# tigert1998/ray-tracing-cuda

Hardware: AMD Instinct MI355X
Metric: Mrays/s (higher is better)
Workload: dtype f32

## Files before the change

### ray-tracing-cuda_amd/csrc/closest_hit.h

```cpp
#pragma once

#ifdef RTMI_CHECK_MARGINS
__device__ inline bool aabb_hit_reference(const BvhNode &nd, V3 o, V3 d, double t_from, double t_to) {
  const float oo[3] = {o.x, o.y, o.z}, dd[3] = {d.x, d.y, d.z};
  for (int i = 0; i < 3; i++) {
    if (dd[i] == 0.f) continue;
    for (int s = 0; s < 2; s++) {
      const float tf = ((s == 0 ? nd.mn[i] : nd.mx[i]) - oo[i]) / dd[i];
      const double t = (double)tf;
      if (t != t || fabs(t) == (double)INFINITY) continue;
      if (!(t_from <= t && t <= t_to)) continue;
      const float pt[3] = {oo[0] + (float)t * dd[0], oo[1] + (float)t * dd[1], oo[2] + (float)t * dd[2]};
      bool inside = true;
      for (int a = 0; a < 3; a++)
        if (a != i && !(nd.mn[a] <= pt[a] && pt[a] <= nd.mx[a])) inside = false;
      if (inside) return true;
    }
  }
  return false;
}
template <typename T>
__device__ inline bool bvh_reference_walk(const SceneDev &sc, const BvhRec &br, V3 o, V3 d, T &t_to, int &face, float &fu,
                                          float &fv) {
  int stk_node[kRefDepthMax + 2], stk_first[kRefDepthMax + 2], stk_n[kRefDepthMax + 2];
  int sp = 1;
  stk_node[0] = br.root, stk_first[0] = 0, stk_n[0] = br.n_faces;
  bool hit = false;
  while (sp > 0) {
    sp--;
    const int node = stk_node[sp], first = stk_first[sp], n = stk_n[sp];
    const BvhNode nd = sc.nodes[node];
    if (node != br.root && !aabb_hit_reference(nd, o, d, 1e-3, (double)t_to)) continue;
    if (nd.right < 0) {
      for (int i = 0; i < n; i++) {
        const int fi = sc.face_of_orig[br.face_base + first + i];
        const FaceRec &f = sc.faces[fi];
        float t = 0.f, u = 0.f, v = 0.f;
        if (tri_test<T>(mk(f.p0[0], f.p0[1], f.p0[2]), mk(f.e1[0], f.e1[1], f.e1[2]), mk(f.e2[0], f.e2[1], f.e2[2]), o, d,
                        t_to, t, u, v))
          t_to = (T)t, face = fi, fu = u, fv = v, hit = true;
      }
    } else if (sp + 2 <= kRefDepthMax + 2) {
      const int mid = (n - 1) / 2;
      stk_node[sp] = nd.right, stk_first[sp] = first + mid + 1, stk_n[sp] = n - mid - 1;
      stk_node[sp + 1] = nd.left, stk_first[sp + 1] = first, stk_n[sp + 1] = mid + 1;
      sp += 2;
    }
  }
  return hit;
}
#endif

template <uint32_t M>
__device__ __forceinline__ bool load_tri_pts(const SceneDev &sc, const float4 *s_tris, int rec, int which, V3 &p0, V3 &e1, V3 &e2) {
  float4 qa, qb, qc;
  bool present;
  if ((M & PIN_LDS_TABLES) || s_tris != nullptr) {
    const float4 *pp = s_tris + (size_t)rec * 3;
    qa = load_lds<float4>(pp), qb = load_lds<float4>(pp + 1), qc = load_lds<float4>(pp + 2);
    present = !(__float_as_int(qc.y) & TRIPTS_ABSENT);
  } else {
    const float4 *pp = reinterpret_cast<const float4 *>(sc.tris + rec);
    qa = load_global<float4>(pp), qb = load_global<float4>(pp + 1), qc = load_global<float4>(pp + 2);
    const float4 qd = load_global<float4>(pp + 3);
    present = which == 0 || (__float_as_int(qd.y) & TRI_SECOND);
  }
  p0 = mk(qa.x, qa.y, qa.z), e1 = mk(qa.w, qb.x, qb.y), e2 = mk(qb.z, qb.w, qc.x);
  return present;
}

template <uint32_t F, bool OCC = false, uint32_t M = 0>
__device__ __forceinline__ Hit closest_hit(const SceneDev &sc, const BvhNode *s_nodes, int lds_nodes, const int *s_paths,
                                           int lds_paths, const float4 *s_tris, int *ll, uint16_t *cands, int *wl,
                                           unsigned long long *overflow, V3 o, V3 d, bool live, bool count_work
#ifdef RTMI_STATS
                                           , MeshStats &st
#endif
                                           , double t_start = INFINITY, double t_stop = INFINITY, bool *uncertain = nullptr
) {
  constexpr bool DT = (F & F_SPHERE) != 0;
  typedef typename TSel<DT>::type T;
  bool ok = false;
  T t_to = OCC ? (T)t_start : (T)INFINITY;
#define RTMI_DECIDED (OCC && ok && t_to <= (T)t_stop)
  uint32_t win = ID_NONE;
  int32_t aux = 0;
  int32_t work = 0;
  float bu = 0.f, bv = 0.f;

  double sa = 0.0, sa2 = 0.0;
  float saf = 0.f;
  if (F & F_SPHERE) {
    float la = len3(d);
    saf = la * la;
    sa = (double)saf;
    sa2 = 2 * sa;
  }

  const int lane = (int)(threadIdx.x & 63u);
  const bool det_safe = (M & PIN_DET_SAFE) || sc.det_safe != 0;
  constexpr bool SLAB = culls_by_slab(M);
  const bool cull_list = (F & F_TRIS) && ((M & PIN_LDS_TABLES) || (ll != nullptr && sc.n_pairs >= kCullMinPairs));
  V3 cull_inv = splat(0.f), cull_klo = splat(0.f), cull_khi = splat(0.f);
  if ((F & F_TRIS) && cull_list) {
    const float ix = __builtin_amdgcn_rcpf(d.x), iy = __builtin_amdgcn_rcpf(d.y), iz = __builtin_amdgcn_rcpf(d.z);
    cull_inv = mk(fabsf(d.x) < 1e-30f ? copysignf(1e30f, d.x) : ix, fabsf(d.y) < 1e-30f ? copysignf(1e30f, d.y) : iy,
                  fabsf(d.z) < 1e-30f ? copysignf(1e30f, d.z) : iz);
    if (SLAB) {
      cull_klo = mk(-o.x * cull_inv.x, -o.y * cull_inv.y, -o.z * cull_inv.z);
    } else {
      const float delta = MESH_DIST_SLACK * (fmaxf(fmaxf(fabsf(o.x), fabsf(o.y)), fabsf(o.z)) + sc.list_mag);
      cull_klo = mk(-(o.x + delta) * cull_inv.x, -(o.y + delta) * cull_inv.y, -(o.z + delta) * cull_inv.z);
      cull_khi = mk(-(o.x - delta) * cull_inv.x, -(o.y - delta) * cull_inv.y, -(o.z - delta) * cull_inv.z);
    }
  }

  for (int ri = 0; ri < sc.n_runs; ri++) {
    if (OCC) {
      live = live && !RTMI_DECIDED;
      if (__builtin_amdgcn_ballot_w64(live) == 0ull) break;
    }
    const i32x4 rv = load_run(sc.runs, ri);
    Run run;
    run.kind = rv[0], run.first = rv[1], run.count = rv[2], run.pad = rv[3];
    if (live && run.kind == RUN_SKY) {
      const T ts = (T)1e9f;
      bool hit = ts <= t_to;
      bool acc = hit && (!ok || ts < t_to);
      ok = ok || acc;
      t_to = acc ? ts : t_to;
      win = acc ? make_id(RUN_SKY, 0) : win;
    }
    if ((F & F_TRIS) && run.kind == RUN_TRIS && cull_list) {
      const int pair0 = run.first >> 1;
      const float lo0 = T_FROM_F * kTimeLo;
      for (int c0 = 0; c0 < run.count; c0 += 32) {
        if (OCC && __builtin_amdgcn_ballot_w64(live && !RTMI_DECIDED) == 0ull) break;
        const int nc = run.count - c0 < 32 ? run.count - c0 : 32;
        const float hi0 = (float)t_to * kTimeHi + kTimeAbs;
        uint32_t mask = 0u;
        RTMI_STAT2(const unsigned long long tc0 = stat_now();)
#define RTMI_CULL_PAIR(bx)                                                                                                      \
  {                                                                                                                             \
    const float t0x = __builtin_fmaf(bx[0], cull_inv.x, cull_klo.x), t1x = __builtin_fmaf(bx[3], cull_inv.x, cull_khi.x); \
    const float t0y = __builtin_fmaf(bx[1], cull_inv.y, cull_klo.y), t1y = __builtin_fmaf(bx[4], cull_inv.y, cull_khi.y); \
    const float t0z = __builtin_fmaf(bx[2], cull_inv.z, cull_klo.z), t1z = __builtin_fmaf(bx[5], cull_inv.z, cull_khi.z); \
    const float en = fmaxf(fmaxf(fminf(t0x, t1x), fminf(t0y, t1y)), fminf(t0z, t1z));                                            \
    const float le = fminf(fminf(fmaxf(t0x, t1x), fmaxf(t0y, t1y)), fmaxf(t0z, t1z));                                            \
    cull_step(mask, fmaxf(lo0, en), fminf(hi0, le));                                                                            \
  }
#define RTMI_CULL_SLAB(bx)                                                                                                      \
  {                                                                                                                             \
    const float tcx = __builtin_fmaf(bx[0], cull_inv.x, cull_klo.x), tcy = __builtin_fmaf(bx[1], cull_inv.y, cull_klo.y),       \
                tcz = __builtin_fmaf(bx[2], cull_inv.z, cull_klo.z);                                                            \
    const float nx = __builtin_fmaf(-bx[3], fabsf(cull_inv.x), tcx), fx = __builtin_fmaf(bx[3], fabsf(cull_inv.x), tcx);        \
    const float ny = __builtin_fmaf(-bx[4], fabsf(cull_inv.y), tcy), fy = __builtin_fmaf(bx[4], fabsf(cull_inv.y), tcy);        \
    const float nz = __builtin_fmaf(-bx[5], fabsf(cull_inv.z), tcz), fz = __builtin_fmaf(bx[5], fabsf(cull_inv.z), tcz);        \
    const float en = fmaxf(fmaxf(nx, ny), nz), le = fminf(fminf(fx, fy), fz);                                                   \
    cull_step_nlt(mask, fminf(hi0, le), fmaxf(lo0, en));                                                                        \
  }
#define RTMI_CULL_ONE(bx)  \
  if (SLAB) RTMI_CULL_SLAB(bx) else RTMI_CULL_PAIR(bx)
        const PairBox *const recs = sc.pair_boxes;
        f32x8 A = load_pair_box(recs, pair0 + c0), B;
        int i = 0;
        for (; i + 1 < nc; i += 2) {
          __builtin_amdgcn_s_waitcnt(0xc07f);
          __builtin_amdgcn_sched_barrier(0);
          B = load_pair_box(recs, pair0 + c0 + i + 1);
          __builtin_amdgcn_sched_barrier(0);
          RTMI_CULL_ONE(A)
          __builtin_amdgcn_s_waitcnt(0xc07f);
          __builtin_amdgcn_sched_barrier(0);
          A = load_pair_box(recs, pair0 + c0 + i + 2);
          __builtin_amdgcn_sched_barrier(0);
          RTMI_CULL_ONE(B)
        }
        if (i < nc) {
          __builtin_amdgcn_s_waitcnt(0xc07f);
          __builtin_amdgcn_sched_barrier(0);
          RTMI_CULL_ONE(A)
        }
#undef RTMI_CULL_ONE
#undef RTMI_CULL_SLAB
#undef RTMI_CULL_PAIR
        mask = __brev(mask) >> (32 - nc);
        if (!live) mask = 0u;
        if (OCC && RTMI_DECIDED) mask = 0u;
        RTMI_STAT2(const unsigned long long tc1 = stat_now(); st.cyc[5] += tc1 - tc0;)
        RTMI_STAT(st.cull_bits += (unsigned)__popcll(__builtin_amdgcn_ballot_w64(true)) * 0u; { unsigned pc = __builtin_popcount(mask); for (int off = 32; off > 0; off >>= 1) pc += __shfl_down(pc, off); st.cull_bits += __builtin_amdgcn_readfirstlane(pc); } st.cull_rays += (unsigned)__popcll(__builtin_amdgcn_ballot_w64(true));)
#ifndef RTMI_OWN_FIRST
#define RTMI_OWN_FIRST 1
#endif
#if RTMI_OWN_FIRST
        if (__builtin_amdgcn_ballot_w64(mask != 0u) != 0ull) {
          if (mask != 0u) {
            const int bit = __builtin_ctz(mask);
            mask &= mask - 1u;
            const int rec = 2 * (pair0 + c0 + bit);
            V3 p0, e1, e2, p1, e1b, e2b;
            (void)load_tri_pts<M>(sc, s_tris, rec, 0, p0, e1, e2);
            const bool second = load_tri_pts<M>(sc, s_tris, rec + 1, 1, p1, e1b, e2b);
            float ta = 0.f, ua = 0.f, va = 0.f, tb = 0.f, ub = 0.f, vb = 0.f;
            const bool hit_a = tri_test_flat<T>(p0, e1, e2, cross3(d, e2), o, d, t_to, ta, ua, va, det_safe);
            bool hit_b = false;
            if (second) hit_b = tri_test_flat<T>(p1, e1b, e2b, cross3(d, e2b), o, d, t_to, tb, ub, vb, det_safe) && !hit_a;
            const float t = hit_a ? ta : tb;
            const bool acc = (hit_a || hit_b) && (!ok || (T)t < t_to);
            ok = ok || acc;
            t_to = acc ? (T)t : t_to;
            win = acc ? make_id(RUN_TRIS, run.first + 2 * (c0 + bit) + (hit_a ? 0 : 1)) : win;
            if (F & F_TEX) {
              bu = acc ? (hit_a ? ua : ub) : bu;
              bv = acc ? (hit_a ? va : vb) : bv;
            }
          }
        }
        if (OCC && RTMI_DECIDED) mask = 0u;
#endif
        {
          constexpr int RW = (F & F_TEX) ? 6 : 2;
          int *tasks = ll + 64 * 8, *results = ll + 64 * 8 + kListTasks(F);
          const int cnt = __builtin_popcount(mask);
          const int base = wave_prefix_excl(cnt);
          if (cnt != 0) {
            int *rr = ll + lane * 8;
            int w3 = 0, w7 = 0;
            if (DT) {
              const double td = (double)t_to;
              w3 = __double2loint(td), w7 = __double2hiint(td);
            } else {
              w3 = __float_as_int((float)t_to);
            }
            *reinterpret_cast<int4 *>(rr) = make_int4(__float_as_int(o.x), __float_as_int(o.y), __float_as_int(o.z), w3);
            *reinterpret_cast<int4 *>(rr + 4) = make_int4(__float_as_int(d.x), __float_as_int(d.y), __float_as_int(d.z), w7);
          }
          bool todo = cnt != 0;
          while (__builtin_amdgcn_ballot_w64(todo) != 0ull) {
            RTMI_STAT(st.cull_iters++;)
            const int lo_t = __builtin_amdgcn_readlane(base, __builtin_ctzll(__builtin_amdgcn_ballot_w64(todo)));
            const bool now = todo && base + cnt - lo_t <= kListTasks(F);
            const int n_now = __builtin_amdgcn_readlane(base + cnt, 63 - __builtin_clzll(__builtin_amdgcn_ballot_w64(now))) - lo_t;
            RTMI_STAT(st.nnow_hist[(n_now - 1) >> 5 < 5 ? (n_now - 1) >> 5 : 5]++;)
            if (now) {
              int k = base - lo_t;
              for (uint32_t m = mask; m != 0u; m &= m - 1u) tasks[k++] = (lane << 5) | __builtin_ctz(m);
            }
            wave_lds_fence();
            for (int t0 = 0; t0 < 2 * n_now; t0 += 64) {
              const int ti = t0 + lane;
              if (ti < 2 * n_now) {
                const int w = tasks[ti >> 1], which = ti & 1;
                const int *orr = ll + (w >> 5) * 8;
                const float4 r0 = *reinterpret_cast<const float4 *>(orr), r1 = *reinterpret_cast<const float4 *>(orr + 4);
                T t0_to;
                if (DT) {
                  t0_to = (T)__hiloint2double(__float_as_int(r1.w), __float_as_int(r0.w));
                } else {
                  t0_to = (T)r0.w;
                }
                const V3 ro = mk(r0.x, r0.y, r0.z), rd = mk(r1.x, r1.y, r1.z);
                V3 p0, e1, e2;
                const bool present = load_tri_pts<M>(sc, s_tris, 2 * (pair0 + c0 + (w & 31)) + which, which, p0, e1, e2);
                float tt = 0.f, uu = 0.f, vv = 0.f;
                bool hit = false;
                if (present) hit = tri_test_flat<T>(p0, e1, e2, cross3(rd, e2), ro, rd, t0_to, tt, uu, vv, det_safe);
                int *res = results + (ti >> 1) * RW;
                res[which] = hit ? __float_as_int(tt) : (int)0xffffffff;
                if (F & F_TEX) res[2 + 2 * which] = __float_as_int(uu), res[3 + 2 * which] = __float_as_int(vv);
              }
            }
            wave_lds_fence();
            RTMI_STAT2(const unsigned long long tc2 = stat_now();)
            if (now) {
              int k = base - lo_t;
              for (uint32_t m = mask; m != 0u; m &= m - 1u, k++) {
                const int tri = run.first + 2 * (c0 + __builtin_ctz(m));
                const int *res = results + k * RW;
                const int ia = res[0], ib = res[1];
                const float ta = __int_as_float(ia), tb = __int_as_float(ib);
                const bool hit_a = ia != (int)0xffffffff && (T)ta <= t_to;
                const bool hit_b = !hit_a && ib != (int)0xffffffff && (T)tb <= t_to;
                const float t = hit_a ? ta : tb;
                const bool acc = (hit_a || hit_b) && (!ok || (T)t < t_to);
                ok = ok || acc;
                t_to = acc ? (T)t : t_to;
                win = acc ? make_id(RUN_TRIS, tri + (hit_a ? 0 : 1)) : win;
                if (F & F_TEX) {
                  bu = acc ? __int_as_float(hit_a ? res[2] : res[4]) : bu;
                  bv = acc ? __int_as_float(hit_a ? res[3] : res[5]) : bv;
                }
              }
              todo = false;
            }
            wave_lds_fence();
            RTMI_STAT2(st.cyc[7] += stat_now() - tc2;)
          }
        }
        RTMI_STAT2(st.cyc[6] += stat_now() - tc1;)
      }
    } else if ((F & F_TRIS) && live && run.kind == RUN_TRIS) {
      const HotTri *base = sc.tris + run.first;
      f32x16 A = load_hot_tri(base, 0);
      for (int i = 0; i < run.count; i++) {
        if (OCC && __builtin_amdgcn_ballot_w64(!RTMI_DECIDED) == 0ull) break;
        __builtin_amdgcn_s_waitcnt(0xc07f);
        __builtin_amdgcn_sched_barrier(0);
        const f32x16 B = load_hot_tri(base, 2 * i + 1);
        __builtin_amdgcn_sched_barrier(0);
        float t = 0.f, u = 0.f, v = 0.f;
        const V3 pv_a = cross3(d, mk(A[6], A[7], A[8]));
        const bool hit_a = tri_test_flat<T>(mk(A[0], A[1], A[2]), mk(A[3], A[4], A[5]), mk(A[6], A[7], A[8]), pv_a, o, d,
                                            t_to, t, u, v, det_safe);
        {
          bool acc = hit_a && (!ok || (T)t < t_to);
          ok = ok || acc;
          t_to = acc ? (T)t : t_to;
          win = acc ? make_id(RUN_TRIS, run.first + 2 * i) : win;
          if (F & F_TEX) {
            bu = acc ? u : bu;
            bv = acc ? v : bv;
          }
        }
        __builtin_amdgcn_s_waitcnt(0xc07f);
        __builtin_amdgcn_sched_barrier(0);
        A = load_hot_tri(base, 2 * i + 2);
        __builtin_amdgcn_sched_barrier(0);
        if (__float_as_int(B[13]) & TRI_SECOND) {
          V3 pv_b = pv_a;
          if (!(__float_as_int(B[13]) & TRI_SAME_E2)) pv_b = cross3(d, mk(B[6], B[7], B[8]));
          bool hit_b = tri_test_flat<T>(mk(B[0], B[1], B[2]), mk(B[3], B[4], B[5]), mk(B[6], B[7], B[8]), pv_b, o, d,
                                        t_to, t, u, v, det_safe);
          hit_b = hit_b && !hit_a;
          bool acc = hit_b && (!ok || (T)t < t_to);
          ok = ok || acc;
          t_to = acc ? (T)t : t_to;
          win = acc ? make_id(RUN_TRIS, run.first + 2 * i + 1) : win;
          if (F & F_TEX) {
            bu = acc ? u : bu;
            bv = acc ? v : bv;
          }
        }
      }
    }
    bool grouped_done = false;
    if ((F & F_SGROUP) && run.kind == RUN_SPHERE && run.pad >= 0 && cands != nullptr) {
      const int n_groups = (run.count + kSphGroupSize - 1) / kSphGroupSize;
      uint16_t *my_cands = cands + lane * kSphCand;
      int *tasks = ll + 64 * 8, *results = ll + 64 * 8 + kListTasks(F);
      int ccnt = 0;
      bool have = false;
      double best_v = 0.0;
      int best_idx = 0;
      {
        int *rr = ll + lane * 8;
        *reinterpret_cast<int4 *>(rr) = make_int4(__float_as_int(o.x), __float_as_int(o.y), __float_as_int(o.z), __float_as_int(saf));
        *reinterpret_cast<int4 *>(rr + 4) = make_int4(__float_as_int(d.x), __float_as_int(d.y), __float_as_int(d.z), 0);
      }
      const float sdelta = kSphDistSlack * fmaxf(fmaxf(fabsf(o.x), fabsf(o.y)), fabsf(o.z));
      const float six = __builtin_amdgcn_rcpf(d.x), siy = __builtin_amdgcn_rcpf(d.y), siz = __builtin_amdgcn_rcpf(d.z);
      const V3 s_inv = mk(fabsf(d.x) < 1e-30f ? copysignf(1e30f, d.x) : six, fabsf(d.y) < 1e-30f ? copysignf(1e30f, d.y) : siy,
                          fabsf(d.z) < 1e-30f ? copysignf(1e30f, d.z) : siz);
      const V3 s_klo = mk(-(o.x + sdelta) * s_inv.x, -(o.y + sdelta) * s_inv.y, -(o.z + sdelta) * s_inv.z);
      const V3 s_khi = mk(-(o.x - sdelta) * s_inv.x, -(o.y - sdelta) * s_inv.y, -(o.z - sdelta) * s_inv.z);
      const float s_lo0 = T_FROM_F * kTimeLo, s_hi0 = (float)t_to * kTimeHi + kTimeAbs;
      const int member0 = __float_as_int(load_sph_group(sc.sph_groups, run.pad)[6]);
      auto flush = [&]() {
        const int cnt = ccnt;
        const int base = wave_prefix_excl(cnt);
        bool todo = cnt != 0;
        while (__builtin_amdgcn_ballot_w64(todo) != 0ull) {
          const int lo_t = __builtin_amdgcn_readlane(base, __builtin_ctzll(__builtin_amdgcn_ballot_w64(todo)));
          const bool now = todo && base + cnt - lo_t <= kListTasks(F);
          const int n_now = __builtin_amdgcn_readlane(base + cnt, 63 - __builtin_clzll(__builtin_amdgcn_ballot_w64(now))) - lo_t;
          if (now)
            for (int j = 0; j < cnt; j++) tasks[base - lo_t + j] = (lane << 16) | (int)my_cands[j];
          wave_lds_fence();
          for (int t0 = 0; t0 < n_now; t0 += 64) {
            const int ti = t0 + lane;
            if (ti < n_now) {
              const int w = tasks[ti];
              const int *orr = ll + (w >> 16) * 8;
              const float4 r0 = *reinterpret_cast<const float4 *>(orr), r1 = *reinterpret_cast<const float4 *>(orr + 4);
              const SphMember *mp = sc.sph_members + member0 + (w & 0xffff);
              const float4 m0 = *reinterpret_cast<const float4 *>(mp);
              const int4 m1 = *reinterpret_cast<const int4 *>(reinterpret_cast<const char *>(mp) + 16);
              const double r2 = __hiloint2double(m1.w, m1.z);
              const V3 ro = mk(r0.x, r0.y, r0.z), rd = mk(r1.x, r1.y, r1.z);
              const double tsa = (double)r0.w, tsa2 = 2 * tsa;
              const V3 oc = ro - mk(m0.x, m0.y, m0.z);
              const double b = (double)(2.0f * dot3(rd, oc));
              const float lc = len3(oc);
              const double c = (double)(lc * lc) - r2;
              const double disc = b * b - 4 * tsa * c;
              double v = __hiloint2double(0x7ff80000, 0);
              if (!(disc < 0)) {
                const double sq = sqrt(disc);
                const double t1 = (-b - sq) / tsa2;
                if (1e-3 <= t1) {
                  v = t1;
                } else {
// ... 386 lines not shown
```

### ray-tracing-cuda_amd/csrc/kernels.h

```cpp
#pragma once
#include <hip/hip_runtime.h>
#include <stdint.h>

#include "../../include/rtmi.h"
#include "scene_dev.h"

#define RTMI_KERNEL_MAX_DEPTH 64

namespace rtmi {

int64_t frame_pixel_of(const FrameDev &fr, int rank, int64_t q);

hipError_t launch_rng_init(uint64_t seed, const FrameDev &fr, const uint32_t *d_jump, uint32_t *d_states,
                           hipStream_t stream, int64_t first = -1);

uint32_t pick_variant(uint32_t features);
int render_occupancy(uint32_t variant, const SceneDev &sc, const FrameDev &fr, int threads, bool fast_path = false);
struct RenderTuning {
  int schedule;
  int blocks_per_cu;
  int threads;
  int sparse_stride;
  int exclusive;
  int outlier_x10;
  int head_pct[3];
  int probe_spp;
  int promote;
  int first_pass;
  int cost_probe;
  int lane_stride;
  int plan;
  int prio_every;
  int fast_path;
  int head_classes;
  int first_prio;
  int fetch_batch, fetch_batch_first;
};

enum : uint32_t {
  PIN_NIBBLE_IDS = 1u << 0,
  PIN_LDS_TABLES = 1u << 1,
  PIN_UNSIGNED = 1u << 2,
  PIN_DET_SAFE = 1u << 3,
  PIN_POW2_FRAME = 1u << 4,
  PIN_EVERY_LANE = 1u << 5,
  PIN_PRIORITIES = 1u << 6,
  PIN_CHAINS = 1u << 7,
  PIN_QUEUE = 1u << 8,
};
constexpr uint32_t kFastCommon = PIN_NIBBLE_IDS | PIN_LDS_TABLES | PIN_UNSIGNED | PIN_DET_SAFE | PIN_POW2_FRAME |
                                 PIN_EVERY_LANE | PIN_PRIORITIES;
constexpr uint32_t kFastChains = kFastCommon | PIN_CHAINS;
constexpr uint32_t kFastQueue = kFastCommon | PIN_QUEUE;
constexpr bool defers_unit(uint32_t m) { return (m & kFastCommon) == kFastCommon; }
constexpr bool culls_by_slab(uint32_t m) { return (m & kFastCommon) == kFastCommon; }
struct FastPathFacts {
  int enabled;
  uint32_t variant;
  int n_mats;
  int mats_in_lds;
  int pairs_in_lds;
  int unsigned_colours;
  int det_safe;
  int width, height;
  int lane_stride;
  int priorities;
  int chains;
  int resumed;
  int tile_cost;
};
uint32_t fast_path_mode(const FastPathFacts &f);
FastPathFacts fast_path_facts(uint32_t variant, const SceneDev &sc, const FrameDev &fr, int threads, int enabled);
bool slab_reach_covers(float list_mag, const CameraDev &cam);
size_t render_lds_bytes(uint32_t variant, const SceneDev &sc, const FrameDev &fr, int threads);
struct SchedPlan {
  const uint32_t *tile_order = nullptr;
  uint32_t *visit_counts = nullptr;
  const uint32_t *sparse_items = nullptr;
  const uint32_t *head_list = nullptr;
  const uint32_t *probe_marks = nullptr;
  int probe_spp = 2;
  uint32_t *prio_tab = nullptr;
  const uint32_t *tile_cost = nullptr;
  const int32_t *chain_next = nullptr;
  const uint32_t *chain_fut = nullptr;
  const int32_t *chain_first = nullptr;
  uint32_t *claims = nullptr;
  int plan_simds = 0, plan_rounds = 0;
};
size_t render_params_bytes();
hipError_t launch_render(uint32_t variant, const SceneDev &sc, const FrameDev &fr, uint32_t *d_states, float *d_out,
                         uint32_t *d_ray_counts, unsigned long long *d_counters, const SchedPlan &plan, bool probe,
                         uint32_t fast, int blocks, int threads, const RenderTuning &tune, void *d_params, hipStream_t stream);
constexpr int kHeadCap = 16384;
hipError_t launch_tile_order(uint32_t *d_ray_counts, int n_tiles, uint32_t *d_cost, uint32_t *d_meta,
                             uint32_t *d_order, uint32_t *d_head, uint32_t sparse_cap, int grid_waves, int outlier_x10,
                             const int head_pct[3], hipStream_t stream);

hipError_t launch_quarter_order(const uint32_t *d_order, const uint32_t *d_work, const uint32_t *d_rays, int n_tiles,
                                uint32_t *d_qcost, uint32_t *d_qsorted, uint32_t *d_qmax, uint32_t *d_qmap, hipStream_t stream);

hipError_t launch_chain_plan(const uint32_t *d_order, const uint32_t *d_cost, int n_tiles, int simds, int rounds, int spp,
                             int probe_spp, int32_t *d_first, int32_t *d_next, uint32_t *d_fut, hipStream_t stream);

hipError_t launch_untile(const FrameDev &fr, const float *d_tiles, float *d_image, hipStream_t stream);
hipError_t launch_untile_u32(const FrameDev &fr, const uint32_t *d_tiles, uint32_t *d_image, hipStream_t stream);
hipError_t launch_post(float *d_img, int64_t n, int spp, hipStream_t stream);
uint32_t pick_query_variant(uint32_t features);
hipError_t launch_query(uint32_t variant, const SceneDev &sc, const QueryDev &qd, int n_cu, int64_t n, const float *d_o,
                        const float *d_d, const float *d_t_max, int32_t *d_hits, unsigned long long *d_abandoned,
                        unsigned long long *d_check, hipStream_t stream);
hipError_t launch_occlusion(uint32_t variant, const SceneDev &sc, const float near_lo[3], const float near_hi[3],
                            float near_short, int n_cu, int64_t n, const float *d_o, const float *d_d,
                            const float *d_t_max, uint8_t *d_occluded, unsigned long long *d_counts,
                            unsigned long long *d_check, hipStream_t stream);
constexpr size_t kCallParamsOffset = 256;
hipError_t launch_trace(uint32_t variant, const SceneDev &sc, bool tex_layers, int n_cu, int64_t n, int max_depth,
                        const float *d_o, const float *d_d, uint32_t *d_states, float *d_radiance,
                        uint32_t *d_ray_counts, unsigned long long *d_work, hipStream_t stream);
hipError_t launch_bounce(uint32_t variant, const SceneDev &sc, const QueryDev &qd, int n_cu, int64_t n, float *d_o, float *d_d,
                         uint32_t *d_states, float *d_emitted, float *d_attenuation, int32_t *d_hits, uint32_t *d_steps,
                         unsigned long long *d_work, hipStream_t stream);
hipError_t launch_path_fold(int64_t n, int layers, const float *d_dirs, const uint32_t *d_steps, const float *d_emitted,
                            const float *d_attenuation, float *d_radiance, hipStream_t stream);
hipError_t launch_budget(uint32_t variant, const SceneDev &sc, bool tex_layers, int n_cu, const FrameDev &fr,
                         const uint32_t *d_budget, uint32_t *d_states, float *d_sum, float *d_sq, uint32_t *d_samples,
                         uint32_t *d_ray_counts, const FeatureBufs *feat, unsigned long long *d_work, hipStream_t stream);
hipError_t launch_resolve_features(const FrameDev &fr, const FeatureBufs &sums, const uint32_t *d_samples,
                                   const FeatureBufs &out, hipStream_t stream);
hipError_t launch_budget_plan(const FrameDev &fr, int min_samples, int max_samples, int step, float tolerance, float floor,
                              const float *d_sum, const float *d_sq, const uint32_t *d_samples, uint32_t *d_budget,
                              unsigned long long *d_totals, hipStream_t stream);
hipError_t launch_resolve(const FrameDev &fr, const float *d_sum, const uint32_t *d_samples, int post, float *d_tiles,
                          hipStream_t stream);
hipError_t launch_resolve_variance(const FrameDev &fr, const float *d_sum, const float *d_sq, const uint32_t *d_samples,
                                   float *d_var, hipStream_t stream);
struct DenoiseCall {
  int height, width, iterations, normal_squarings, demodulate;
  float sigma_color, sigma_depth;
  const float *color, *variance, *albedo, *normal, *depth, *alpha;
  float *out, *out_variance;
  void *scratch;
};
size_t denoise_scratch_bytes(int height, int width);
hipError_t launch_denoise(const DenoiseCall &d, hipStream_t stream);
struct AccumulateCall {
  int height, width;
  float normal_min, depth_tolerance, min_blend;
  float e[3], h[3], v[3], p[3];
  float prev_p[3], r[3][3];
  const float *color, *variance, *normal, *depth, *alpha;
  const void *history_in;
  void *history_out;
  float *out, *out_variance, *out_length;
};
size_t history_bytes(int height, int width);
hipError_t launch_accumulate(const AccumulateCall &c, hipStream_t stream);
hipError_t launch_camera_rays(const FrameDev &fr, const CameraDev &cam, const float w[3], int kind, float fov,
                              const uint32_t *d_budget, uint32_t sample, uint32_t *d_states, float *d_origins,
                              float *d_dirs, hipStream_t stream);
hipError_t launch_sample_add(const FrameDev &fr, const uint32_t *d_budget, uint32_t sample, const float *d_radiance,
                             const uint32_t *d_trace_counts, float *d_sum, float *d_sq, uint32_t *d_samples,
                             uint32_t *d_ray_counts, hipStream_t stream);
#ifdef RTMI_STATS
hipError_t copy_wave_stats(unsigned long long *host, size_t bytes);
#endif
#ifdef RTMI_CHECK_MARGINS
hipError_t launch_add_one(unsigned long long *d_word, hipStream_t stream);
#endif
hipError_t launch_arithmetic_selftest(unsigned long long *d_bad, hipStream_t stream);

}
```

### ray-tracing-cuda_amd/csrc/mesh_search.h

```cpp
#pragma once

__device__ __forceinline__ int lane_rank(unsigned long long mask) {
  return (int)__builtin_amdgcn_mbcnt_hi((unsigned)(mask >> 32), __builtin_amdgcn_mbcnt_lo((unsigned)mask, 0u));
}
__device__ __forceinline__ int wave_prefix_excl(int v) {
  int s = v;
  s += __builtin_amdgcn_update_dpp(0, s, 0x111, 0xf, 0xf, true);
  s += __builtin_amdgcn_update_dpp(0, s, 0x112, 0xf, 0xf, true);
  s += __builtin_amdgcn_update_dpp(0, s, 0x114, 0xf, 0xf, true);
  s += __builtin_amdgcn_update_dpp(0, s, 0x118, 0xf, 0xf, true);
  s += __builtin_amdgcn_update_dpp(0, s, 0x142, 0xa, 0xf, false);
  s += __builtin_amdgcn_update_dpp(0, s, 0x143, 0xc, 0xf, false);
  return s - v;
}
__device__ __forceinline__ void wave_lds_fence() {
  __builtin_amdgcn_fence(__ATOMIC_ACQ_REL, "wavefront");
  __builtin_amdgcn_wave_barrier();
}
__device__ __forceinline__ float ubyte_f32(uint32_t x, int byte) { return (float)((x >> (8 * byte)) & 0xffu); }

#ifndef MESH_DIST_SLACK
#define MESH_DIST_SLACK kDistSlack
#endif

struct NodeFrame {
  float ka[3], kb[3], idq[3];
};
__device__ __forceinline__ void node_frame(uint4 w0, float4 r0, float4 r2, float mag, NodeFrame &f) {
  const float delta = MESH_DIST_SLACK * (fmaxf(fmaxf(fabsf(r0.x), fabsf(r0.y)), fabsf(r0.z)) + mag);
  const float oo[3] = {r0.x, r0.y, r0.z}, ii[3] = {r2.x, r2.y, r2.z};
  const float org[3] = {__uint_as_float(w0.x), __uint_as_float(w0.y), __uint_as_float(w0.z)};
#ifdef RTMI_NO_SLACK_EXP
  const int sk = 0;
#else
  const int sk = (int)w0.w >> 24;
#endif
#pragma unroll
  for (int a = 0; a < 3; a++) {
    const int ex = (int)(int8_t)((w0.w >> (8 * a)) & 0xffu);
    const float oq = ldexpf(oo[a] - org[a], -ex);
    const float rho = ldexpf(delta, sk - ex);
    f.idq[a] = __builtin_amdgcn_fmed3f(ldexpf(ii[a], ex), -1e35f, 1e35f);
    f.ka[a] = -(oq + rho) * f.idq[a];
    f.kb[a] = -(oq - rho) * f.idq[a];
  }
}
__device__ __forceinline__ bool child_box_hit(const NodeFrame &f, float qlx, float qly, float qlz, float qhx, float qhy,
                                              float qhz, float lo0, float hi0) {
  const float ql[3] = {qlx, qly, qlz}, qh[3] = {qhx, qhy, qhz};
  float en = -INFINITY, le = INFINITY;
#pragma unroll
  for (int a = 0; a < 3; a++) {
    const float tl = __builtin_fmaf(ql[a], f.idq[a], f.ka[a]);
    const float th = __builtin_fmaf(qh[a], f.idq[a], f.kb[a]);
    en = fmaxf(en, fminf(tl, th));
    le = fminf(le, fmaxf(tl, th));
  }
  const float lo = fmaxf(lo0, __builtin_fmaf(-fabsf(en), kSlabTimeRel, en));
  const float hi = fminf(hi0, __builtin_fmaf(fabsf(le), kSlabTimeRel, le));
  return lo <= hi;
}

__device__ __forceinline__ void hit_list_insert(const SceneDev &sc, int *rr, uint32_t code, int face, int orig,
                                                float t) {
  const int cnt = rr[12];
  const uint32_t cut = (uint32_t)rr[13], lo_code = (uint32_t)rr[14];
  if (!(code >= lo_code && code < cut)) return;
  int found = -1, jmax = 0;
  uint32_t cmax = 0u;
#pragma unroll
  for (int j = 0; j < kHitSlots; j++) {
    if (j < cnt) {
      const uint32_t cj = (uint32_t)rr[16 + j * kHitWords];
      if (cj == code) found = j;
      if (cj >= cmax) cmax = cj, jmax = j;
    }
  }
  int slot = -1;
  if (found >= 0) {
    const float tj = __int_as_float(rr[16 + found * kHitWords + 2]);
    bool better = t < tj;
    if (t == tj) better = orig > sc.faces[rr[16 + found * kHitWords + 1]].orig;
    if (better) slot = found;
  } else if (cnt < kHitSlots) {
    slot = cnt;
    rr[12] = cnt + 1;
  } else if (code > cmax) {
    rr[13] = (int)code;
  } else {
    rr[13] = (int)cmax;
    slot = jmax;
  }
  if (slot >= 0) {
    rr[16 + slot * kHitWords] = (int)code;
    rr[16 + slot * kHitWords + 1] = face;
    rr[16 + slot * kHitWords + 2] = __float_as_int(t);
  }
}

#ifdef RTMI_STATS
struct MeshStats {
  unsigned searches, node_steps, face_steps, nodes_popped, blocks_popped, insert_rounds, steps_hist[6];
  unsigned long long cull_bits, cull_rays, cull_iters;
  unsigned nnow_hist[6];
  unsigned long long calib;
  unsigned long long cyc[11];
};
__device__ unsigned long long g_wave_stats[16384][16];
__device__ __forceinline__ unsigned long long stat_real() {
  __builtin_amdgcn_sched_barrier(0);
  unsigned long long t;
  asm volatile("s_waitcnt vmcnt(0) lgkmcnt(0)\n\ts_memtime %0\n\ts_waitcnt lgkmcnt(0)" : "=s"(t)::"memory");
  __builtin_amdgcn_sched_barrier(0);
  return t;
}
#if RTMI_STATS == 9
__device__ __forceinline__ unsigned long long stat_now() { return 0ull; }
#else
__device__ __forceinline__ unsigned long long stat_now() { return stat_real(); }
#endif
#define RTMI_STAT(x) x
#if RTMI_STATS == 2
#define RTMI_STAT2(x) x
#else
#define RTMI_STAT2(x)
#endif
#if RTMI_STATS == 3
#define RTMI_STAT3(x) x
#else
#define RTMI_STAT3(x)
#endif
#else
#define RTMI_STAT(x)
#define RTMI_STAT2(x)
#define RTMI_STAT3(x)
#endif

template <typename T, bool DT>
__device__ __forceinline__ void mesh_search(const SceneDev &sc, int sub_root, const BvhNode *top, float mag, int *wl,
                                            bool need, V3 o, V3 d, V3 inv_d, T bt_to, uint32_t lo_code,
                                            unsigned long long *overflow, bool count_work
#ifdef RTMI_STATS
                                            , MeshStats &st
#endif
) {
  const int lane = (int)(threadIdx.x & 63u);
  RTMI_STAT(st.searches++; unsigned my_steps = 0; const unsigned long long tset0 = stat_now();)
  int *stack = wl + 64 * kMeshRayWords;
  const float lo0 = T_FROM_F * kTimeLo;
  if (need) {
    int *rr = wl + lane * kMeshRayWords;
    int w3 = 0, w7 = 0;
    if (DT) {
      const double td = (double)bt_to;
      w3 = __double2loint(td), w7 = __double2hiint(td);
    } else {
      w3 = __float_as_int((float)bt_to);
    }
    *reinterpret_cast<int4 *>(rr + 0) = make_int4(__float_as_int(o.x), __float_as_int(o.y), __float_as_int(o.z), w3);
    *reinterpret_cast<int4 *>(rr + 4) = make_int4(__float_as_int(d.x), __float_as_int(d.y), __float_as_int(d.z), w7);
    *reinterpret_cast<int4 *>(rr + 8) = make_int4(__float_as_int(inv_d.x), __float_as_int(inv_d.y), __float_as_int(inv_d.z),
                                                  __float_as_int((float)bt_to * kTimeHi + kTimeAbs));
    *reinterpret_cast<int4 *>(rr + 12) = make_int4(0, (int)kCodeNone, (int)lo_code, 0);
  }
  const unsigned long long nm = __ballot(need);
  const int reserve = sc.sub_reserve;
  int sn = 0, sf = 0;
  if (__popcll(nm) <= kTopRays) {
    const BvhNode te = top[lane];
    const float far = (float)bt_to * kTimeHi + kTimeAbs;
    for (unsigned long long m = nm; m != 0ull; m &= m - 1ull) {
      const int rl = __builtin_ctzll(m);
      if (kMeshStackWords - sn - sf - reserve < kTopEntries) {
        if (lane == 0) stack[sn] = (rl << 26) | sub_root;
        sn++;
        continue;
      }
      const V3 ro = mk(__int_as_float(__builtin_amdgcn_readlane(__float_as_int(o.x), rl)),
                       __int_as_float(__builtin_amdgcn_readlane(__float_as_int(o.y), rl)),
                       __int_as_float(__builtin_amdgcn_readlane(__float_as_int(o.z), rl)));
      const V3 ri = mk(__int_as_float(__builtin_amdgcn_readlane(__float_as_int(inv_d.x), rl)),
                       __int_as_float(__builtin_amdgcn_readlane(__float_as_int(inv_d.y), rl)),
                       __int_as_float(__builtin_amdgcn_readlane(__float_as_int(inv_d.z), rl)));
      const float rfar = __int_as_float(__builtin_amdgcn_readlane(__float_as_int(far), rl));
      const float delta = ldexpf(MESH_DIST_SLACK * (fmaxf(fmaxf(fabsf(ro.x), fabsf(ro.y)), fabsf(ro.z)) + mag), te.right);
      const bool hit = te.left != -1 && slab_touch(te, delta, ro, ri, lo0, rfar);
      const bool pn = hit && te.left >= 0, pf = hit && te.left < 0;
      const unsigned long long mn_ = __builtin_amdgcn_ballot_w64(pn), mf_ = __builtin_amdgcn_ballot_w64(pf);
      const uint32_t owner_bits = (uint32_t)rl << 26;
      if (pn) stack[sn + lane_rank(mn_)] = (int)(owner_bits | (uint32_t)te.left);
      if (pf) stack[kMeshStackWords - 1 - sf - lane_rank(mf_)] = (int)(owner_bits | (uint32_t)(-(te.left + 1)));
      sn += __popcll(mn_);
      sf += __popcll(mf_);
    }
  } else {
    if (need) stack[lane_rank(nm)] = (lane << 26) | sub_root;
    sn = __popcll(nm);
  }
  wave_lds_fence();
  RTMI_STAT(unsigned long long tprev = stat_now(); st.cyc[9] += tprev - tset0;
            { const unsigned long long cb = stat_now(); st.calib += cb - tprev; tprev = cb; } (void)tprev;)
  while ((sn | sf) != 0) {
    if (sf >= 64 || sn == 0) {
      const bool wide = sf <= 16, pair = !wide && sf <= 32;
      const int kf = sf < 64 ? sf : 64;
      RTMI_STAT(st.face_steps++; st.blocks_popped += kf; my_steps++;)
      RTMI_STAT2(const unsigned long long tf0 = stat_now(); st.cyc[10] += tf0 - tprev;)
      const int slot = wide ? (lane >> 2) : pair ? (lane >> 1) : lane;
      const bool mine = slot < kf;
      const int fstride = pair ? 2 : 1;
      int e = 0;
      if (mine) e = stack[kMeshStackWords - sf + slot];
      sf -= kf;
      wave_lds_fence();
      unsigned pend = 0u;
      float pt0 = 0.f, pt1 = 0.f, pt2 = 0.f, pt3 = 0.f;
      float po0 = 0.f, po1 = 0.f, po2 = 0.f, po3 = 0.f, pc0 = 0.f, pc1 = 0.f, pc2 = 0.f, pc3 = 0.f;
      const int owner = (int)((unsigned)e >> 26), fcnt = e & 7;
      int first = (e >> 3) & (kMeshMaxFaces - 1);
      int *rr = wl + owner * kMeshRayWords;
      if (!DT && count_work && mine) atomicAdd(rr + 7, 1);
      if (wide) {
        const int j = lane & 3;
        first += j;
        if (mine && j < fcnt) {
          const float4 r0 = *reinterpret_cast<const float4 *>(rr + 0), r1 = *reinterpret_cast<const float4 *>(rr + 4);
          T t_to;
          if (DT) {
            t_to = (T)__hiloint2double(__float_as_int(r1.w), __float_as_int(r0.w));
          } else {
            t_to = (T)r0.w;
          }
          const float4 *fp4 = reinterpret_cast<const float4 *>(sc.faces + first);
          const float4 a = fp4[0], b = fp4[1], c = fp4[2];
          float t = 0.f, u = 0.f, v = 0.f;
          bool th = tri_test<T>(mk(a.x, a.y, a.z), mk(a.w, b.x, b.y), mk(b.z, b.w, c.x), mk(r0.x, r0.y, r0.z),
                                mk(r1.x, r1.y, r1.z), t_to, t, u, v);
#if defined(RTMI_ABLATE) && RTMI_ABLATE == 2
          th = th && t < -1.f;
#endif
          if (th) pend = 1u, pt0 = t, po0 = c.y, pc0 = c.w;
        }
      } else if (pair) {
        first += lane & 1;
        if (mine) {
          const float4 r0 = *reinterpret_cast<const float4 *>(rr + 0), r1 = *reinterpret_cast<const float4 *>(rr + 4);
          T t_to;
          if (DT) {
            t_to = (T)__hiloint2double(__float_as_int(r1.w), __float_as_int(r0.w));
          } else {
            t_to = (T)r0.w;
          }
          const V3 ro = mk(r0.x, r0.y, r0.z), rd = mk(r1.x, r1.y, r1.z);
          const float4 *fp4 = reinterpret_cast<const float4 *>(sc.faces + first);
          const int left = fcnt - (lane & 1);
          float4 q[6];
#pragma unroll
// ... 196 lines not shown
```

### ray-tracing-cuda_amd/csrc/render_body.h

```cpp
#pragma once

struct QueryHit;
template <uint32_t F>
__device__ __forceinline__ QueryHit resolve_hit(const SceneDev &sc, const QueryDev &qd, const Hit &h, V3 o, V3 d);

struct LaunchCfg {
  int32_t lds_mats;
  int32_t wide_ids;
  int32_t stack_off;
  int32_t nodes_off;
  int32_t lds_nodes;
  int32_t mesh_off;
  int32_t exclusive;
  int32_t pairs_off;
  int32_t list_off;
  int32_t paths_off;
  int32_t lds_paths;
  int32_t threads;
  int32_t nrm_off;
  int32_t probe_spp;
  int32_t promote;
  int32_t cand_off;
  const uint32_t *tile_order;
  uint32_t *visit_counts;
// ... 737 lines not shown
                const uint32_t at = ids_offset(depth >> 1);
                const uint32_t old = smem[at];
                smem[at] = (uint8_t)((depth & 1) ? ((old & 0x0fu) | ((uint32_t)mat << 4)) : ((old & 0xf0u) | (uint32_t)mat));
              } else if (lc.wide_ids) {
                *reinterpret_cast<uint16_t *>(smem + ids_offset(depth)) = (uint16_t)mat;
              } else {
                smem[ids_offset(depth)] = (uint8_t)mat;
              }
              depth++;
              if (DEFER && m.kind == MAT_LAMBERTIAN) depth |= kOwesBit;
              o = p;
              d = nd;
              ended = false;
            }
          }
        }
      }
      RTMI_STAT2(if (!(F & F_BVH)) { const unsigned long long tsb = stat_now();
        if ((int)(threadIdx.x & 63u) == __builtin_ctzll(__ballot(1))) g_wave_stats[((blockIdx.x * blockDim.x + threadIdx.x) >> 6) & 16383u][10] += tsb - tq2; })
      if constexpr (STEP) {
        const int64_t q = (int64_t)q32;
        float *em = step->emitted + q * 3, *at = step->attenuation + q * 3, *dr = step->dirs + q * 3;
        em[0] = result.x, em[1] = result.y, em[2] = result.z;
        at[0] = step_att.x, at[1] = step_att.y, at[2] = step_att.z;
        dr[0] = step_d.x, dr[1] = step_d.y, dr[2] = step_d.z;
        if (!ended) {
          float *on = step->origins + q * 3;
          on[0] = step_o.x, on[1] = step_o.y, on[2] = step_o.z;
          states[0 * n_items + q] = rng.d;
          states[1 * n_items + q] = rng.v0;
          states[2 * n_items + q] = rng.v1;
          states[3 * n_items + q] = rng.v2;
          states[4 * n_items + q] = rng.v3;
          states[5 * n_items + q] = rng.v4;
        }
        if (step->hits) {
          const auto r = resolve_hit<F>(sc, step->qd, h, o, d);
          int4 *rec = reinterpret_cast<int4 *>(step->hits + q * 12);
          rec[0] = make_int4(__float_as_int(r.t), __float_as_int(r.u), __float_as_int(r.v), __float_as_int(r.n.x));
          rec[1] = make_int4(__float_as_int(r.n.y), __float_as_int(r.n.z), r.mat, r.kind);
          rec[2] = make_int4(r.entry, r.element, 0, 0);
        }
        if (step->steps) step->steps[q] += 1u;
        ray_acc += 1u;
        active = false, has_px = false;
        ended = false;
      }
      if (ended) {
        int i = depth - 1;
        if (!tex32 && fast_fold) {
          const uint32_t step = n_threads;
          if (nibble_ids) {
            uint32_t at = ids_offset(i >= 0 ? i >> 1 : 0);
            if (i >= 0 && !(i & 1)) {
              const int m0 = lds_byte(at) & 15;
              { const V3 a_ = lds_rgb(m0); result = mk(a_.x * result.x, a_.y * result.y, a_.z * result.z); }
              i--, at -= step;
            }
            for (; i >= 3; i -= 4, at -= 2u * step) {
              const uint32_t b0 = lds_byte(at), b1 = lds_byte(at - step);
              const int m0 = b0 >> 4, m1 = b0 & 15, m2 = b1 >> 4, m3 = b1 & 15;
              const V3 a0 = lds_rgb(m0), a1 = lds_rgb(m1);
              const V3 a2 = lds_rgb(m2), a3 = lds_rgb(m3);
              result = mk(a0.x * result.x, a0.y * result.y, a0.z * result.z);
              result = mk(a1.x * result.x, a1.y * result.y, a1.z * result.z);
              result = mk(a2.x * result.x, a2.y * result.y, a2.z * result.z);
              result = mk(a3.x * result.x, a3.y * result.y, a3.z * result.z);
            }
            for (; i >= 1; i -= 2, at -= step) {
              const uint32_t b0 = lds_byte(at);
              const int m0 = b0 >> 4, m1 = b0 & 15;
              { const V3 a_ = lds_rgb(m0); result = mk(a_.x * result.x, a_.y * result.y, a_.z * result.z); }
              { const V3 a_ = lds_rgb(m1); result = mk(a_.x * result.x, a_.y * result.y, a_.z * result.z); }
            }
          } else {
            uint32_t at = ids_offset(i >= 0 ? i : 0);
            for (; i >= 3; i -= 4, at -= 4u * step) {
              const int m0 = lds_byte(at), m1 = lds_byte(at - step), m2 = lds_byte(at - 2u * step), m3 = lds_byte(at - 3u * step);
              const V3 a0 = lds_rgb(m0), a1 = lds_rgb(m1);
              const V3 a2 = lds_rgb(m2), a3 = lds_rgb(m3);
              result = mk(a0.x * result.x, a0.y * result.y, a0.z * result.z);
              result = mk(a1.x * result.x, a1.y * result.y, a1.z * result.z);
              result = mk(a2.x * result.x, a2.y * result.y, a2.z * result.z);
              result = mk(a3.x * result.x, a3.y * result.y, a3.z * result.z);
            }
            for (; i >= 0; i--, at -= step) {
              const int m0 = lds_byte(at);
              { const V3 a_ = lds_rgb(m0); result = mk(a_.x * result.x, a_.y * result.y, a_.z * result.z); }
            }
          }
        }
        for (; !FOLD4 && i >= 0; i--) {
          V3 a;
          if (tex32) {
            const uint32_t lw = *reinterpret_cast<const uint32_t *>(smem + tex_layer_offset(i));
            if (lw >> 31) {
              a = texel_rgb(lw);
            } else if (mats_in_lds) {
              a = lds_rgb((int)lw);
            } else {
              a = mk(sc.mats[lw].r, sc.mats[lw].g, sc.mats[lw].b);
            }
          } else {
            const int mi = nibble_ids     ? (int)((smem[ids_offset(i >> 1)] >> ((i & 1) * 4)) & 15u)
                           : lc.wide_ids ? (int)*reinterpret_cast<const uint16_t *>(smem + ids_offset(i))
                                         : (int)smem[ids_offset(i)];
            if (mats_in_lds) {
              a = lds_rgb(mi);
            } else {
              a = mk(sc.mats[mi].r, sc.mats[mi].g, sc.mats[mi].b);
            }
          }
          if (sc.unsigned_colours) {
            result = mk(a.x * result.x, a.y * result.y, a.z * result.z);
          } else {
            result = mk(0.f + a.x * result.x, 0.f + a.y * result.y, 0.f + a.z * result.z);
          }
        }
        color = color + result;
        if constexpr (BUDGET)
          moment = mk(__fadd_rn(moment.x, __fmul_rn(result.x, result.x)), __fadd_rn(moment.y, __fmul_rn(result.y, result.y)),
                      __fadd_rn(moment.z, __fmul_rn(result.z, result.z)));
        active = false;
      }
    }
    RTMI_STAT(st.cyc[4] += stat_now() - tq2;)
  }

  if (RTMI_PRIO) wave_priority_leave(lc.prio_tab);
#undef RTMI_CHAINS
#undef RTMI_PRIO
  {
    unsigned long long ray_total = ray_acc;
    for (int off = 32; off > 0; off >>= 1) ray_total += __shfl_down(ray_total, off);
    if ((threadIdx.x & 63) == 0 && ray_total) atomicAdd(&counters[1], ray_total);
  }
#ifdef RTMI_STATS
  if (!QUEUE && (threadIdx.x & 63) == 0) {
    const unsigned v[13] = {wave_queries, st.searches, st.node_steps, st.face_steps, st.nodes_popped, st.blocks_popped,
                            st.insert_rounds, st.steps_hist[0], st.steps_hist[1], st.steps_hist[2], st.steps_hist[3],
                            st.steps_hist[4], st.steps_hist[5]};
    for (int i = 0; i < 13; i++) atomicAdd(&counters[4 + i], (unsigned long long)v[i]);
    for (int i = 0; i < 9; i++) atomicAdd(&counters[17 + i], st.cyc[i]);
    const unsigned long long life = stat_real() - t_begin;
    atomicAdd(&counters[26], life);
    atomicMax(&counters[27], life);
    atomicAdd(&counters[28], 1ull);
    atomicAdd(&counters[29], st.calib);
    atomicAdd(&counters[30], st.cull_bits);
    atomicAdd(&counters[31], st.cull_iters);
    atomicAdd(&counters[32], st.cull_rays);
    for (int i = 0; i < 3; i++)
      atomicAdd(&counters[37 + i], (unsigned long long)st.nnow_hist[2 * i] | ((unsigned long long)st.nnow_hist[2 * i + 1] << 32));
    const unsigned wid = (blockIdx.x * blockDim.x + threadIdx.x) >> 6;
    if (!(F & F_BVH) && wid < 16384u) {
      atomicAdd(&counters[25], g_wave_stats[wid][9]);
      atomicAdd(&counters[6], g_wave_stats[wid][10]);
      g_wave_stats[wid][9] = 0, g_wave_stats[wid][10] = 0;
      g_wave_stats[wid][0] = life, g_wave_stats[wid][11] = wave_queries;
      g_wave_stats[wid][12] = t_begin_rt, g_wave_stats[wid][13] = __builtin_amdgcn_s_memrealtime();
      g_wave_stats[wid][14] = (unsigned long long)__builtin_amdgcn_s_getreg(0xF804) | ((unsigned long long)__builtin_amdgcn_s_getreg(0xF814) << 32);
    } else if (wid < 16384u) {
      g_wave_stats[wid][0] = life;
#if RTMI_STATS != 9
      for (int i = 0; i < 9; i++) g_wave_stats[wid][1 + i] = st.cyc[i];
#endif
      g_wave_stats[wid][10] = wave_queries, g_wave_stats[wid][11] = st.node_steps, g_wave_stats[wid][12] = st.face_steps;
      g_wave_stats[wid][13] = st.nodes_popped, g_wave_stats[wid][14] = st.insert_rounds;
      g_wave_stats[wid][15] = (st.cyc[9] << 32) | (st.cyc[10] >> 8);
    }
  }
#endif
}
```

Before: 35670.

## Fold per-ray closest triangle hit with wave-scoped LDS atomic min

In the fast-path cull-list loop, each lane tests one triangle of a pair, resolves the pair with a DPP swap, and folds the winning (t, slot) into a per-ray 64-bit key with an LDS atomic min. Each ray then reads its key back and accepts the hit in one step. The aim is to replace the ordered per-ray reduction over tasks. When a tie or ordering case is flagged, it falls back to the original ordered loop and bumps an overflow counter. It also adds a stats-only histogram of per-ray trip counts.

```diff
diff --git a/ray-tracing-cuda_amd/csrc/closest_hit.h b/ray-tracing-cuda_amd/csrc/closest_hit.h
--- a/ray-tracing-cuda_amd/csrc/closest_hit.h
+++ b/ray-tracing-cuda_amd/csrc/closest_hit.h
@@ -100,6 +100,8 @@
   const int lane = (int)(threadIdx.x & 63u);
   const bool det_safe = (M & PIN_DET_SAFE) || sc.det_safe != 0;
   constexpr bool SLAB = culls_by_slab(M);
+  constexpr bool MINF = folds_by_min(M);
+  static_assert(!MINF || (!OCC && !DT && !(F & F_TEX)), "a key holds a binary32 t and the triangle's place, nothing else");
   const bool cull_list = (F & F_TRIS) && ((M & PIN_LDS_TABLES) || (ll != nullptr && sc.n_pairs >= kCullMinPairs));
   V3 cull_inv = splat(0.f), cull_klo = splat(0.f), cull_khi = splat(0.f);
   if ((F & F_TRIS) && cull_list) {
@@ -242,11 +244,61 @@
             const bool now = todo && base + cnt - lo_t <= kListTasks(F);
             const int n_now = __builtin_amdgcn_readlane(base + cnt, 63 - __builtin_clzll(__builtin_amdgcn_ballot_w64(now))) - lo_t;
             RTMI_STAT(st.nnow_hist[(n_now - 1) >> 5 < 5 ? (n_now - 1) >> 5 : 5]++;)
+            RTMI_STAT({
+              int pc = now ? cnt : 0;
+              for (int off = 32; off > 0; off >>= 1) pc = max(pc, __shfl_xor(pc, off));
+              st.trip_hist[pc < 8 ? pc - 1 : 7]++;
+            })
+            int ln = lane;
+            if (MINF) asm volatile("" : "+v"(ln));
             if (now) {
               int k = base - lo_t;
               for (uint32_t m = mask; m != 0u; m &= m - 1u) tasks[k++] = (lane << 5) | __builtin_ctz(m);
+              if (MINF) results[2 * ln + 1] = -1;
             }
             wave_lds_fence();
+            if (MINF) {
+              bool flagged = false;
+              for (int t0 = 0; t0 < 2 * n_now; t0 += 64) {
+                const int ti = t0 + ln;
+                if (ti < 2 * n_now) {
+                  const int w = tasks[ti >> 1], which = ti & 1;
+                  const int *orr = ll + (w >> 5) * 8;
+                  const float4 r0 = *reinterpret_cast<const float4 *>(orr), r1 = *reinterpret_cast<const float4 *>(orr + 4);
+                  const V3 ro = mk(r0.x, r0.y, r0.z), rd = mk(r1.x, r1.y, r1.z);
+                  V3 p0, e1, e2;
+                  const bool present = load_tri_pts<M>(sc, s_tris, 2 * (pair0 + c0 + (w & 31)) + which, which, p0, e1, e2);
+                  float tt = 0.f, uu, vv;
+                  bool hit = false;
+                  if (present) hit = tri_test_flat<T>(p0, e1, e2, cross3(rd, e2), ro, rd, (T)r0.w, tt, uu, vv, det_safe);
+                  const int mine = hit ? __float_as_int(tt) : -1;
+                  const int other = __builtin_amdgcn_update_dpp(mine, mine, 0xb1, 0xf, 0xf, false);
+                  const bool yield = other != -1 && (which != 0 || __int_as_float(other) < tt);
+                  flagged = flagged || (hit && yield && which == 0);
+                  if (hit && !yield) {
+                    const unsigned long long key = ((unsigned long long)(uint32_t)mine << 32) | (uint32_t)(2 * (w & 31) + which);
+                    (void)__hip_atomic_fetch_min(reinterpret_cast<unsigned long long *>(results + 2 * (w >> 5)), key,
+                                                 __ATOMIC_RELAXED, __HIP_MEMORY_SCOPE_WAVEFRONT);
+                  }
+                }
+              }
+              wave_lds_fence();
+              const unsigned long long fl = __builtin_amdgcn_ballot_w64(flagged);
+              if (fl == 0ull) {
+                if (now) {
+                  const int2 key = *reinterpret_cast<const int2 *>(results + 2 * ln);
+                  const float t = __int_as_float(key.y);
+                  const bool acc = key.y != -1 && (!ok || (T)t < t_to);
+                  ok = ok || acc;
+                  t_to = acc ? (T)t : t_to;
+                  win = acc ? make_id(RUN_TRIS, run.first + 2 * c0 + key.x) : win;
+                  todo = false;
+                }
+                wave_lds_fence();
+                continue;
+              }
+              if (lane == 0) atomicAdd(overflow + (kOrderedTasksWord - 2), (unsigned long long)__popcll(fl));
+            }
             for (int t0 = 0; t0 < 2 * n_now; t0 += 64) {
               const int ti = t0 + lane;
               if (ti < 2 * n_now) {
diff --git a/ray-tracing-cuda_amd/csrc/kernels.h b/ray-tracing-cuda_amd/csrc/kernels.h
--- a/ray-tracing-cuda_amd/csrc/kernels.h
+++ b/ray-tracing-cuda_amd/csrc/kernels.h
@@ -54,6 +54,8 @@
 constexpr uint32_t kFastQueue = kFastCommon | PIN_QUEUE;
 constexpr bool defers_unit(uint32_t m) { return (m & kFastCommon) == kFastCommon; }
 constexpr bool culls_by_slab(uint32_t m) { return (m & kFastCommon) == kFastCommon; }
+constexpr bool folds_by_min(uint32_t m) { return (m & kFastCommon) == kFastCommon; }
+constexpr int kOrderedTasksWord = 16;
 struct FastPathFacts {
   int enabled;
   uint32_t variant;
diff --git a/ray-tracing-cuda_amd/csrc/mesh_search.h b/ray-tracing-cuda_amd/csrc/mesh_search.h
--- a/ray-tracing-cuda_amd/csrc/mesh_search.h
+++ b/ray-tracing-cuda_amd/csrc/mesh_search.h
@@ -103,6 +103,7 @@
   unsigned searches, node_steps, face_steps, nodes_popped, blocks_popped, insert_rounds, steps_hist[6];
   unsigned long long cull_bits, cull_rays, cull_iters;
   unsigned nnow_hist[6];
+  unsigned trip_hist[8];
   unsigned long long calib;
   unsigned long long cyc[11];
 };
diff --git a/ray-tracing-cuda_amd/csrc/render_body.h b/ray-tracing-cuda_amd/csrc/render_body.h
--- a/ray-tracing-cuda_amd/csrc/render_body.h
+++ b/ray-tracing-cuda_amd/csrc/render_body.h
@@ -913,6 +913,8 @@
     atomicAdd(&counters[32], st.cull_rays);
     for (int i = 0; i < 3; i++)
       atomicAdd(&counters[37 + i], (unsigned long long)st.nnow_hist[2 * i] | ((unsigned long long)st.nnow_hist[2 * i + 1] << 32));
+    for (int i = 0; i < 4 && !(F & F_BVH); i++)
+      atomicAdd(&counters[12 + i], (unsigned long long)st.trip_hist[2 * i] | ((unsigned long long)st.trip_hist[2 * i + 1] << 32));
     const unsigned wid = (blockIdx.x * blockDim.x + threadIdx.x) >> 6;
     if (!(F & F_BVH) && wid < 16384u) {
       atomicAdd(&counters[25], g_wave_stats[wid][9]);
```

Measured after the change: 37060, median of 6. 3.9% higher.
